# ningyu1991/InclusiveGAN

Hardware: AMD Instinct MI355X
Metric: training img/sec (whole node), CelebA 128x128 StyleGAN2+IMLE (higher is better)
Workload: dtype f32-equivalent (3x3 convs: 2-piece fp16 split, operands to <= 1 ulp of fp32, scales per pixel / per channel: no per-tensor window; fp32 sums)

## Files before the change

### include/igan_hip.h

```cpp
#ifndef IGAN_HIP_H
#define IGAN_HIP_H

#include <stddef.h>
#include <stdint.h>

#ifdef __cplusplus
extern "C" {
#endif

#define IGAN_ABI_VERSION 10

typedef void* igan_stream_t;

enum igan_status {
    IGAN_OK = 0,
    IGAN_ERR_INVALID_ARGUMENT = 1,
    IGAN_ERR_HIP = 2,
    IGAN_ERR_UNSUPPORTED = 3
};

int igan_abi_version(void);
size_t igan_struct_size(int which);
const char* igan_last_error(void);

// ... 89 lines not shown
    float* workspace;
    size_t workspace_floats;
    int N, H, W, Cin;
    int OH, OW, Cout;
    int KH, KW;
    int stride, up;
    int pad_y, pad_x;
    int splits;
    float alpha;
    const void* x_pieces;
    const void* dy_pieces;
    size_t x_pieces_bytes;
    size_t dy_pieces_bytes;
    const float* x_colmax;
    const float* dy_colmax;
} igan_conv2d_wgrad_params;

int igan_conv2d_wgrad_plan(const igan_conv2d_wgrad_params* p, int* splits, size_t* workspace_floats);
int igan_conv2d_wgrad(igan_stream_t stream, const igan_conv2d_wgrad_params* p);
int igan_conv2d_wgrad_kernel_name(const igan_conv2d_wgrad_params* p, char* buf, int buflen);

int igan_conv_pieces_wanted(int KH, int KW, int Cin, int Cout);
int igan_pieces_image_ok(int N, int HW, int C);
int igan_conv_piece_form(void);
size_t igan_filter_image_bytes(int KH, int KW, int Cin, int Cout);
int igan_filter_image(igan_stream_t stream, const float* w, void* out, int KH, int KW, int Cin, int Cout, int w_transposed);
#define IGAN_FILTER_MAX_GROUPS 48
typedef struct igan_filter_image_desc { const float* w; void* out; int KH, KW, Cin, Cout, w_transposed; } igan_filter_image_desc;
int igan_filter_images_grouped(igan_stream_t stream, const igan_filter_image_desc* groups, int count);
int igan_debug_filter_image_launches(unsigned long long* out, int reset);
size_t igan_colmax_floats(int N, int HW, int C);
int igan_debug_f16_window(unsigned long long* below, unsigned long long* imaged, int reset);
int igan_debug_f16_window_by_kind(unsigned long long* out4, int reset);

int igan_to_pieces(igan_stream_t stream, const float* x, const float* scale, void* out, int N, int HW, int C);

enum { IGAN_DENSE_PRO_NONE = 0, IGAN_DENSE_PRO_SQUARE = 1, IGAN_DENSE_PRO_DEMOD_GRAD = 2 };
enum { IGAN_DENSE_EPI_SCALE = 0, IGAN_DENSE_EPI_BIAS = 1, IGAN_DENSE_EPI_RSQRT = 2, IGAN_DENSE_EPI_STYLE_GRAD = 3 };
typedef struct igan_dense_params {
    const float* x;
    const float* x2;
    const float* w;
    float* y;
    const float* bias;
    const float* e1;
    const float* e2;
    float* colsum;
    int ldx, ldy;
    int M, K, N;
    int w_transposed;
    int prologue, epilogue;
    float alpha, pro_scale, bias_scale, add_const, eps;
} igan_dense_params;
int igan_dense_small(igan_stream_t stream, const igan_dense_params* p);

typedef struct igan_dense_wgrad_params {
    const float* a;
    const float* b;
    const float* b2;
    float* dw;
    int lda;
    int M, K, N;
    int pro_a, pro_b;
    float alpha, pro_scale;
} igan_dense_wgrad_params;
int igan_dense_small_wgrad(igan_stream_t stream, const igan_dense_wgrad_params* p);
// ... 192 lines not shown
```

### inclusivegan_amd/_abi.py

```python
import ctypes
import os
import threading

_HERE = os.path.dirname(os.path.abspath(__file__))
LIB_PATH = os.environ.get('IGAN_LIB') or os.path.join(_HERE, 'csrc', 'libigan_hip.so')

IGAN_OK = 0
IGAN_ERR_INVALID_ARGUMENT = 1
IGAN_ERR_HIP = 2
IGAN_ERR_UNSUPPORTED = 3

c_float_p = ctypes.POINTER(ctypes.c_float)


class UpFirDn2DParams(ctypes.Structure):
    _fields_ = [
        ('x', ctypes.c_void_p), ('k', ctypes.c_void_p), ('y', ctypes.c_void_p),
        ('upx', ctypes.c_int), ('upy', ctypes.c_int), ('downx', ctypes.c_int), ('downy', ctypes.c_int),
        ('padx0', ctypes.c_int), ('padx1', ctypes.c_int), ('pady0', ctypes.c_int), ('pady1', ctypes.c_int),
        ('majorDim', ctypes.c_int), ('inH', ctypes.c_int), ('inW', ctypes.c_int), ('minorDim', ctypes.c_int),
        ('kernelH', ctypes.c_int), ('kernelW', ctypes.c_int),
        ('outH', ctypes.c_int), ('outW', ctypes.c_int),
    ]

# ... 104 lines not shown

DENSE_MAX_GROUPS = 24
FILTER_MAX_GROUPS = 48
DENSE_PRO_NONE, DENSE_PRO_SQUARE, DENSE_PRO_DEMOD_GRAD = 0, 1, 2
DENSE_EPI_SCALE, DENSE_EPI_BIAS, DENSE_EPI_RSQRT, DENSE_EPI_STYLE_GRAD = 0, 1, 2, 3
DENSE_PRO_MUL = 3
DENSE_EPI_DEMOD_GRAD2, DENSE_EPI_STYLE_GRAD2 = 4, 5

_I, _F, _P, _SZ, _LL = ctypes.c_int, ctypes.c_float, ctypes.c_void_p, ctypes.c_size_t, ctypes.c_longlong

SIGNATURES = {
    'igan_abi_version': (_I, []),
    'igan_struct_size': (_SZ, [_I]),
    'igan_last_error': (ctypes.c_char_p, []),
    'igan_upfirdn2d': (_I, [_P, ctypes.POINTER(UpFirDn2DParams)]),
    'igan_upfirdn2d_f16': (_I, [_P, ctypes.POINTER(UpFirDn2DParams)]),
    'igan_upfirdn2d_ban': (_I, [_P, _P, _P, _P, _I, _P, _I, _F, _F]),
    'igan_fused_bias_act': (_I, [_P, ctypes.POINTER(FusedBiasActParams)]),
    'igan_fused_bias_act_f16': (_I, [_P, ctypes.POINTER(FusedBiasActParams)]),
    'igan_bias_grad_workspace_floats': (_SZ, [_I, _I, _I]),
    'igan_bias_grad': (_I, [_P, _P, _P, _P, _I, _I, _I]),
    'igan_bias_act_noise_workspace_floats': (_SZ, [_I, _I]),
    'igan_bias_act_noise_fwd': (_I, [_P, _P, _P, _P, _P, _P, _I, _I, _I, _F, _F]),
    'igan_bias_act_noise_dd_workspace_floats': (ctypes.c_size_t, [_I, _I, _I]),
    'igan_bias_act_noise_bwd_dd': (_I, [_P, _P, _P, _P, _P, _P, _P, _P, _P, _P, _P, _P, _I, _I, _I, _I, _I, _F, _F]),
    'igan_bias_act_noise_bwd': (_I, [_P, _P, _P, _P, _P, _P, _P, _P, _I, _I, _I, _F, _F]),
    'igan_conv2d_plan': (_I, [ctypes.POINTER(Conv2DParams), ctypes.POINTER(_I), ctypes.POINTER(_I), ctypes.POINTER(_SZ)]),
    'igan_conv2d': (_I, [_P, ctypes.POINTER(Conv2DParams)]),
    'igan_conv2d_kernel_name': (_I, [ctypes.POINTER(Conv2DParams), ctypes.c_char_p, _I]),
    'igan_conv2d_wgrad_kernel_name': (_I, [ctypes.POINTER(Conv2DWgradParams), ctypes.c_char_p, _I]),
    'igan_conv2d_wgrad_plan': (_I, [ctypes.POINTER(Conv2DWgradParams), ctypes.POINTER(_I), ctypes.POINTER(_SZ)]),
    'igan_conv2d_wgrad': (_I, [_P, ctypes.POINTER(Conv2DWgradParams)]),
    'igan_debug_f16_window_by_kind': (_I, [_P, _I]),
    'igan_colmax_floats': (ctypes.c_size_t, [_I, _I, _I]),
    'igan_filter_image_bytes': (ctypes.c_size_t, [_I, _I, _I, _I]),
    'igan_filter_image': (_I, [_P, _P, _P, _I, _I, _I, _I, _I]),
    'igan_filter_images_grouped': (_I, [_P, ctypes.POINTER(FilterImageDesc), _I]),
    'igan_debug_filter_image_launches': (_I, [_P, _I]),
    'igan_to_pieces': (_I, [_P, _P, _P, _P, _I, _I, _I]),
    'igan_conv_pieces_wanted': (_I, [_I, _I, _I, _I]),
    'igan_pieces_image_ok': (_I, [_I, _I, _I]),
    'igan_conv_piece_form': (_I, []),
    'igan_debug_f16_window': (_I, [_P, _P, _I]),
    'igan_dense_small': (_I, [_P, ctypes.POINTER(DenseParams)]),
    'igan_dense_small_wgrad': (_I, [_P, ctypes.POINTER(DenseWgradParams)]),
    'igan_dense_small_grouped': (_I, [_P, ctypes.POINTER(DenseParams), _I]),
    'igan_dense_small_wgrad_grouped': (_I, [_P, ctypes.POINTER(DenseWgradParams), _I]),
    'igan_dense_small2_grouped': (_I, [_P, ctypes.POINTER(Dense2Params), _I]),
    'igan_dense_small_wgrad2_grouped': (_I, [_P, ctypes.POINTER(DenseWgrad2Params), _I]),
    'igan_rows_group_sum': (_I, [_P, _P, ctypes.POINTER(ctypes.c_int), _I, _P, _I, _I, _I]),
    'igan_scale_add': (_I, [_P, _P, _P, _P, _P, _P, _I, _I, _I]),
    'igan_sumsq_taps_grouped': (_I, [_P, ctypes.POINTER(TapsParams), _I]),
    'igan_bcast_mul_taps_grouped': (_I, [_P, ctypes.POINTER(TapsParams), _I]),
    'igan_sumsq_taps': (_I, [_P, _P, _P, _I, _I]),
    'igan_bcast_mul_taps': (_I, [_P, _P, _P, _P, _I, _I, _F]),
    'igan_scale_dot_workspace_floats': (_SZ, [_I, _I, _I]),
    'igan_scale_dot': (_I, [_P, _P, _P, _P, _P, _P, _P, _I, _I, _I]),
    'igan_lpips_layer_blocks': (_I, [_I, _I]),
    'igan_lpips_layer_fwd': (_I, [_P, _P, _P, _P, _P, _I, _I, _I]),
    'igan_lpips_layer_bwd': (_I, [_P, _P, _P, _P, _P, _P, _I, _I, _I]),
    'igan_lpips_pairs_fwd': (_I, [_P, _P, _P, _P, _P, _P, _P, _I, _I, _I, _I, _I]),
    'igan_lpips_pairs_bwd': (_I, [_P, _P, _P, _P, _P, _P, _P, _P, _I, _I, _I, _I]),
    'igan_maxpool2x2_fwd': (_I, [_P, _P, _P, _I, _I, _I, _I]),
    'igan_maxpool2x2_bwd': (_I, [_P, _P, _P, _P, _P, _I, _I, _I, _I]),
    'igan_mbstd_workspace_floats': (_SZ, [_I, _I, _I, _I, _I]),
    'igan_mbstd_fwd': (_I, [_P, _P, _P, _P, _I, _I, _I, _I, _I]),
# ... 89 lines not shown
```

### inclusivegan_amd/csrc/conv2d_mfma.hip

```cpp
#include "igan_common.h"
#include <atomic>
#include <cmath>
#include <cstdlib>
#include <type_traits>

namespace {

typedef float f32x16 __attribute__((ext_vector_type(16)));

constexpr int BK = 32;
constexpr int LEAD_STEPS = 8;
constexpr int LDK = BK + 4;

struct ConvArgs {
    const float* x;
    const float* w;
    float* y;
    float* out;
    const float* in_scale;
    const float* out_scale;
    int N, H, W, Cin;
    int OH, OW, Cout;
    int KH, KW;
    int stride, up_shift;
    int pad_y, pad_x;
    int splits;
    int full_tiles;
    int nx, ny;
    int cpt;
    int Mtot;
    int vecA, vecB, vecS;
    int vecY;
    float alpha;
    int xcd_remap;
    int b_scale;
    int prio;
    int walk;
    int stagger;
    unsigned long long* diag;
    const float* bias;
    int act;
    float act_alpha, act_gain;
    const float* noise;
    const float* noise_strength;
    int noise_bcast;
    int diag_mode;
    const unsigned short* xp;
    const unsigned short* wp;
};

__device__ __forceinline__ float noise_term(const ConvArgs& a, int pix) {
    if (a.noise == nullptr || pix < 0) return 0.0f;
    return a.noise[a.noise_bcast ? pix % (a.OH * a.OW) : pix] * a.noise_strength[0];
}

__device__ __forceinline__ float epi_act(int act, float v, float alpha) {
    if (act == 2) return v > 0.f ? v : 0.f;
    if (act == 3) return v > 0.f ? v : v * alpha;
    return v;
}

__device__ __forceinline__ float4 f4zero() { return make_float4(0.f, 0.f, 0.f, 0.f); }
__device__ __forceinline__ float4 f4mul(float4 a, float4 b) { return make_float4(a.x * b.x, a.y * b.y, a.z * b.z, a.w * b.w); }
__device__ __forceinline__ float4 f4sel(bool has, float4 s) { return make_float4(has ? s.x : 1.f, has ? s.y : 1.f, has ? s.z : 1.f, has ? s.w : 1.f); }

typedef unsigned int u32x4 __attribute__((ext_vector_type(4)));
constexpr unsigned OOB = 0x7FFFFFF0u;

__device__ __forceinline__ __amdgpu_buffer_rsrc_t make_rsrc(const float* p, unsigned bytes) {
    return __builtin_amdgcn_make_buffer_rsrc(const_cast<float*>(p), 0, (int)bytes, 0x00020000);
}

struct LoadAddr {
    unsigned off;
    int left;
};
template <bool VEC>
__device__ __forceinline__ LoadAddr make_addr(int off, int left) {
    LoadAddr a;
    if constexpr (VEC) { a.off = (left > 0) ? (unsigned)off * 4u : OOB; a.left = 0; }
    else { a.off = (unsigned)off * 4u; a.left = left; }
// ... 890 lines not shown
    o[1] = __builtin_bit_cast(unsigned short, p1);
}

__device__ __forceinline__ void load_unit16(const float* __restrict__ x, const float* __restrict__ scale, int p, int c, int C, int HW, float (&v)[16]) {
    const float4* src = reinterpret_cast<const float4*>(x + (size_t)p * C + 16 * c);
#pragma unroll
    for (int i = 0; i < 4; i++) { const float4 f = src[i]; v[4 * i] = f.x; v[4 * i + 1] = f.y; v[4 * i + 2] = f.z; v[4 * i + 3] = f.w; }
    if (scale != nullptr) {
        const float4* sc = reinterpret_cast<const float4*>(scale + (size_t)(p / HW) * C + 16 * c);
#pragma unroll
        for (int i = 0; i < 4; i++) { const float4 f = sc[i]; v[4 * i] *= f.x; v[4 * i + 1] *= f.y; v[4 * i + 2] *= f.z; v[4 * i + 3] *= f.w; }
    }
}
__device__ __forceinline__ void store_units(const unsigned short (&pc)[2][16], uint4* stage, unsigned short* __restrict__ out, int total, int chunk) {
#pragma unroll
    for (int q = 0; q < 2; q++)
#pragma unroll
        for (int hh = 0; hh < 2; hh++) {
            uint4 u;
            u.x = pc[q][8 * hh + 0] | ((unsigned)pc[q][8 * hh + 1] << 16); u.y = pc[q][8 * hh + 2] | ((unsigned)pc[q][8 * hh + 3] << 16);
            u.z = pc[q][8 * hh + 4] | ((unsigned)pc[q][8 * hh + 5] << 16); u.w = pc[q][8 * hh + 6] | ((unsigned)pc[q][8 * hh + 7] << 16);
            stage[threadIdx.x * 4 + 2 * q + hh] = u;
        }
    __syncthreads();
    const int units = min(256, total - chunk * 256);
    uint4* dst = reinterpret_cast<uint4*>(out + (size_t)chunk * 256 * 32);
#pragma unroll
    for (int k = 0; k < 4; k++) {
        const int j = k * 256 + threadIdx.x;
        if (j < units * 4) dst[j] = stage[j];
    }
}

__global__ __launch_bounds__(256) void rows_f16_kernel(const float* __restrict__ x, const float* __restrict__ scale, unsigned short* __restrict__ out,
                                                        float* __restrict__ rowinv, float* __restrict__ colmax, int total, int cpp, int lcpp, int C, int HW) {
    __shared__ uint4 stage[256 * 4];
    const int c = threadIdx.x & (cpp - 1);
    float cm[16];
#pragma unroll
    for (int i = 0; i < 16; i++) cm[i] = 0.0f;
    int below = 0;
    const int nchunks = (total + 255) >> 8;
    for (int chunk = blockIdx.x; chunk < nchunks; chunk += gridDim.x) {
        const bool mine = chunk * 256 + (int)threadIdx.x < total;
        const int idx = min(chunk * 256 + (int)threadIdx.x, total - 1);
        const int p = idx >> lcpp;
        float v[16];
        load_unit16(x, scale, p, c, C, HW, v);
        float m = 0.0f;
#pragma unroll
        for (int i = 0; i < 16; i++) { const float av = fabsf(v[i]); m = fmaxf(m, av); if (mine) cm[i] = fmaxf(cm[i], av); }
        for (int o = 1; o < cpp; o <<= 1) m = fmaxf(m, __shfl_xor(m, o));
        const float S = scale_from_amax(m);
        if (mine && c == 0) rowinv[p] = inv_scale_from_amax(m);
        unsigned short pc[2][16];
#pragma unroll
        for (int i = 0; i < 16; i++) {
            unsigned short o[2];
            const float vs = v[i] * S;
            split2(vs, o);
            pc[0][i] = o[0]; pc[1][i] = o[1];
            below += (mine && vs != 0.0f && fabsf(vs) < 0x1p-12f) ? 1 : 0;
        }
        if (chunk != (int)blockIdx.x) __syncthreads();
        store_units(pc, stage, out, total, chunk);
    }
    count_window(below, &g_f16_below_window);
    if (blockIdx.x == 0 && threadIdx.x == 0) atomicAdd(&g_f16_imaged, (unsigned long long)total * 16ull);
    if (colmax != nullptr) {
        __syncthreads();
        float* sm = reinterpret_cast<float*>(stage);
#pragma unroll
        for (int i = 0; i < 16; i++) sm[threadIdx.x * 16 + i] = cm[i];
        __syncthreads();
        const int groups = 256 >> lcpp;
        for (int ch = threadIdx.x; ch < C; ch += 256) {
            const int cc = ch >> 4, i = ch & 15;
            float m = 0.0f;
            for (int j = 0; j < groups; j++) m = fmaxf(m, sm[(j * cpp + cc) * 16 + i]);
            colmax[4 + (size_t)blockIdx.x * C + ch] = m;
        }
        if (blockIdx.x == 0 && threadIdx.x == 0) colmax[0] = (float)gridDim.x;
    }
}

__global__ __launch_bounds__(256) void cols_amax_kernel(const float* __restrict__ x, const float* __restrict__ scale, float* __restrict__ partial,
                                                         int P_, int C4, int lC4, int HW, float* __restrict__ header) {
    if (header != nullptr && blockIdx.x == 0 && threadIdx.x == 0) header[0] = (float)gridDim.x;
    __shared__ float4 red[256];
    const int q = threadIdx.x & (C4 - 1), pl = threadIdx.x >> lC4, ppi = 256 >> lC4;
    const int step = gridDim.x * ppi;
    float4 m = make_float4(0.f, 0.f, 0.f, 0.f);
    auto take = [&](int p) {
        float4 v = reinterpret_cast<const float4*>(x)[(size_t)p * C4 + q];
        if (scale != nullptr) {
            const float4 f = reinterpret_cast<const float4*>(scale)[(size_t)(p / HW) * C4 + q];
            v.x *= f.x; v.y *= f.y; v.z *= f.z; v.w *= f.w;
        }
// ... 232 lines not shown
    const int py = cls >> a.up_shift, px = cls & (up - 1);
    const int QH = (a.OH - py + up - 1) >> a.up_shift;
    const int QW = (a.OW - px + up - 1) >> a.up_shift;
    const int Mcls = a.N * QH * QW;
    const int m0 = mt * BM;
    if (m0 >= Mcls) return;
    const int n0 = nt * BN;
    const int ky0 = (a.pad_y - py * a.stride) & (up - 1);
    const int kx0 = (a.pad_x - px * a.stride) & (up - 1);
    const int nky = (ky0 < a.KH) ? ((a.KH - ky0 + up - 1) >> a.up_shift) : 0;
    const int nkx = (kx0 < a.KW) ? ((a.KW - kx0 + up - 1) >> a.up_shift) : 0;
    const int chunks = nky * nkx * a.cpt;
    const int c_begin = sliced ? (int)(((long long)split * chunks) / nsplit) : 0;
    const int c_end = sliced ? (int)(((long long)(split + 1) * chunks) / nsplit) : chunks;

    const float inv_hw = 1.0f / (float)(QH * QW), inv_w = 1.0f / (float)QW;
    const int drow = 32 * (wave & 3) + (lane >> 1);
    const int dhalf = (lane & 1) ^ ((drow >> 3) & 1);
    const bool lowave = wave < 4;
    const int ntap = nky * nkx;
    int ld_cc, ld_t0;
    if constexpr (TAPO) {
        ld_t0 = (c_begin < c_end) ? c_begin / a.cpt : 0;
        ld_cc = (c_begin < c_end) ? c_begin - ld_t0 * a.cpt : 0;
    } else {
        ld_cc = (c_begin < c_end) ? c_begin / ntap : 0;
        ld_t0 = (c_begin < c_end) ? c_begin - ld_cc * ntap : 0;
    }
    int ld_ta = (c_begin < c_end) ? ld_t0 / nkx : 0;
    int ld_tb = (c_begin < c_end) ? ld_t0 - ld_ta * nkx : 0;
    const unsigned xbytes = (unsigned)a.N * a.H * a.W * a.Cin * (2u * NP), wbytes = (unsigned)a.KH * a.KW * a.Cin * a.Cout * (2u * NP);
    const __amdgpu_buffer_rsrc_t rx = __builtin_amdgcn_make_buffer_rsrc(const_cast<unsigned short*>(a.xp), 0, (int)xbytes, 0x00020000);
    const __amdgpu_buffer_rsrc_t rw = __builtin_amdgcn_make_buffer_rsrc(const_cast<unsigned short*>(a.wp), 0, (int)wbytes, 0x00020000);
    const unsigned pixA = (unsigned)a.Cin * (2u * NP);
    unsigned baseA, maskA = 0u, voffB;
    {
        const int m = m0 + drow;
        const bool rok = m < Mcls;
        const int mm = rok ? m : 0;
        const int nn = div_small(mm, QH * QW, inv_hw);
        const int r = mm - nn * (QH * QW);
        const int qy = div_small(r, QW, inv_w), qx = r - qy * QW;
        const int vy0 = (qy * up + py) * a.stride - a.pad_y + ky0, vx0 = (qx * up + px) * a.stride - a.pad_x + kx0;
        const int iy0 = vy0 >> a.up_shift, ix0 = vx0 >> a.up_shift;
        baseA = (unsigned)((nn * a.H + iy0) * a.W + ix0) * pixA + (unsigned)dhalf * 16u;
        for (int ta = 0; ta < nky; ta++)
            for (int tb = 0; tb < nkx; tb++) {
                const int iy = iy0 + ta, ix = ix0 + tb;
                const bool ok = rok & (iy >= 0) & (ix >= 0) & (iy < a.H) & (ix < a.W);
                maskA |= ok ? (1u << (ta * nkx + tb)) : 0u;
            }
        const int co = n0 + drow;
        voffB = (co < a.Cout) ? (unsigned)co * PB + (unsigned)dhalf * 16u : OOB;
    }
    unsigned offA = OOB, soffB = 0u;
    typedef __attribute__((address_space(3))) void lds_void;
    unsigned char* dA = nullptr;
    bool dma_fresh = true;
    const unsigned sliceB = (unsigned)(a.KH * a.KW * a.Cout) * PB;
    auto dma_prep = [&](int stage) {
        if (!TAPO || dma_fresh || ld_cc == 0) {
            const unsigned disp = (unsigned)(ld_ta * a.W + ld_tb) * pixA + (unsigned)ld_cc * PB;
            const unsigned bit = 1u << (ld_ta * nkx + ld_tb);
            offA = (maskA & bit) ? baseA + disp : OOB;
            const int ky = ky0 + (ld_ta << a.up_shift), kx = kx0 + (ld_tb << a.up_shift);
            soffB = __builtin_amdgcn_readfirstlane((unsigned)((ld_cc * (a.KH * a.KW) + ky * a.KW + kx) * a.Cout) * PB);
            dma_fresh = false;
        } else {
            offA += PB;
            soffB = __builtin_amdgcn_readfirstlane(soffB + sliceB);
        }
        dA = smem + stage * STAGE + (wave & 3) * 1024;
        if constexpr (TAPO) {
            ++ld_cc;
            const int w1 = (ld_cc == a.cpt) ? 1 : 0;
            ld_cc = w1 ? 0 : ld_cc;
            ld_tb += w1;
            const int w2 = (ld_tb == nkx) ? 1 : 0;
            ld_tb = w2 ? 0 : ld_tb;
            ld_ta += w2;
        } else {
            ++ld_tb;
            const int w1 = (ld_tb == nkx) ? 1 : 0;
            ld_tb = w1 ? 0 : ld_tb;
            ld_ta += w1;
            const int w2 = (ld_ta == nky) ? 1 : 0;
            ld_ta = w2 ? 0 : ld_ta;
            ld_cc += w2;
        }
    };
    auto dma_piece = [&](int j) {
        unsigned char* A = dA;
        unsigned char* B = dA + IMG;
        if constexpr (NP == 2) {
            const unsigned sB = __builtin_amdgcn_readfirstlane(soffB);
            if (lowave) {
                if (j == 0) __builtin_amdgcn_raw_ptr_buffer_load_lds(rx, (lds_void*)A, 16, offA, 0, 0, 0);
                if (j == 1) __builtin_amdgcn_raw_ptr_buffer_load_lds(rw, (lds_void*)(B + 4096), 16, voffB, sB + 32u, 0, 0);
            } else {
                if (j == 0) __builtin_amdgcn_raw_ptr_buffer_load_lds(rx, (lds_void*)(A + 4096), 16, offA, 32, 0, 0);
                if (j == 1) __builtin_amdgcn_raw_ptr_buffer_load_lds(rw, (lds_void*)B, 16, voffB, sB, 0, 0);
            }
        } else
        if (lowave) {
            if (j == 0) __builtin_amdgcn_raw_ptr_buffer_load_lds(rx, (lds_void*)A, 16, offA, 0, 0, 0);
            if (j == 1) __builtin_amdgcn_raw_ptr_buffer_load_lds(rx, (lds_void*)(A + 2 * 4096), 16, offA, 64, 0, 0);
            if (j == 2) __builtin_amdgcn_raw_ptr_buffer_load_lds(rw, (lds_void*)(B + 4096), 16, voffB, soffB + 32u, 0, 0);
        } else {
            if (j == 0) __builtin_amdgcn_raw_ptr_buffer_load_lds(rx, (lds_void*)(A + 4096), 16, offA, 32, 0, 0);
            if (j == 1) __builtin_amdgcn_raw_ptr_buffer_load_lds(rw, (lds_void*)B, 16, voffB, soffB, 0, 0);
            if (j == 2) __builtin_amdgcn_raw_ptr_buffer_load_lds(rw, (lds_void*)(B + 2 * 4096), 16, voffB, soffB + 64u, 0, 0);
        }
    };
    auto dma_chunk = [&](int stage) { dma_prep(stage); dma_piece(0); dma_piece(1); if constexpr (NP == 3) dma_piece(2); };

    f32x16 acc[TM];
#pragma unroll
    for (int tm = 0; tm < TM; tm++)
#pragma unroll
        for (int r = 0; r < 16; r++) acc[tm][r] = 0.0f;

    float tabv[3] = {0.0f, 0.0f, 0.0f};
    if constexpr (NP == 2) {
        const float* rowinv = reinterpret_cast<const float*>(reinterpret_cast<const unsigned char*>(a.xp) + (size_t)a.N * a.H * a.W * a.Cin * 4);
#pragma unroll
        for (int j = 0; j < 3; j++) {
            const int i = tid + 512 * j;
            const int t = i >> 7, r = i & 127;
            if (t < ntap) {
                const int ta = t / nkx, tb = t - ta * nkx;
                const int m = m0 + r;
                const bool rok = m < Mcls;
                const int mm = rok ? m : 0;
                const int nn = div_small(mm, QH * QW, inv_hw);
                const int rr = mm - nn * (QH * QW);
                const int qy = div_small(rr, QW, inv_w), qx = rr - qy * QW;
                const int iy = (((qy * up + py) * a.stride - a.pad_y + ky0) >> a.up_shift) + ta, ix = (((qx * up + px) * a.stride - a.pad_x + kx0) >> a.up_shift) + tb;
                if (rok & (iy >= 0) & (ix >= 0) & (iy < a.H) & (ix < a.W)) tabv[j] = rowinv[(nn * a.H + iy) * a.W + ix];
            }
        }
    }
    if (c_begin < c_end) { dma_chunk(0); dma_chunk(1); }
// ... 491 lines not shown
    const bool sliced = bid >= a.full_tiles;
    const int tail = bid - a.full_tiles;
    const int tile = sliced ? a.full_tiles + tail / a.splits : bid;
    const int split = sliced ? tail % a.splits : 0;
    const int nsplit = sliced ? a.splits : 1;
    const int mt = tile % a.nx, nt = (tile / a.nx) % a.ny, cls = tile / (a.nx * a.ny);
    const int py = cls >> a.up_shift, px = cls & (up - 1);
    const int QH = (a.OH - py + up - 1) >> a.up_shift;
    const int QW = (a.OW - px + up - 1) >> a.up_shift;
    const int Mcls = a.N * QH * QW;
    const int m0 = mt * BM;
    if (m0 >= Mcls) return;
    const int n0 = nt * BN;
    const int ky0 = (a.pad_y - py * a.stride) & (up - 1);
    const int kx0 = (a.pad_x - px * a.stride) & (up - 1);
    const int nky = (ky0 < a.KH) ? ((a.KH - ky0 + up - 1) >> a.up_shift) : 0;
    const int nkx = (kx0 < a.KW) ? ((a.KW - kx0 + up - 1) >> a.up_shift) : 0;
    const int chunks = nky * nkx * a.cpt;
    const int c_begin = sliced ? (int)(((long long)split * chunks) / nsplit) : 0;
    const int c_end = sliced ? (int)(((long long)(split + 1) * chunks) / nsplit) : chunks;
    const bool any = c_begin < c_end;

    const float inv_hw = 1.0f / (float)(QH * QW), inv_w = 1.0f / (float)QW;
    const int drow = 32 * wave + (lane >> 1);
    const int dhalf = (lane & 1) ^ ((drow >> 3) & 1);
    const int ntap = nky * nkx;
    int ld_t0 = any ? c_begin / a.cpt : 0;
    int ld_cc = any ? c_begin - ld_t0 * a.cpt : 0;
    int ld_ta = any ? ld_t0 / nkx : 0;
    int ld_tb = any ? ld_t0 - ld_ta * nkx : 0;
    const unsigned xbytes = (unsigned)a.N * a.H * a.W * a.Cin * 4u, wbytes = (unsigned)a.KH * a.KW * a.Cin * a.Cout * 4u;
    const __amdgpu_buffer_rsrc_t rx = __builtin_amdgcn_make_buffer_rsrc(const_cast<unsigned short*>(a.xp), 0, (int)xbytes, 0x00020000);
    const __amdgpu_buffer_rsrc_t rw = __builtin_amdgcn_make_buffer_rsrc(const_cast<unsigned short*>(a.wp), 0, (int)wbytes, 0x00020000);
    const unsigned pixA = (unsigned)a.Cin * 4u;
    unsigned baseA, maskA = 0u, voffB;
    {
        const int m = m0 + drow;
        const bool rok = m < Mcls;
        const int mm = rok ? m : 0;
        const int nn = div_small(mm, QH * QW, inv_hw);
        const int r = mm - nn * (QH * QW);
        const int qy = div_small(r, QW, inv_w), qx = r - qy * QW;
        const int vy0 = (qy * up + py) * a.stride - a.pad_y + ky0, vx0 = (qx * up + px) * a.stride - a.pad_x + kx0;
        const int iy0 = vy0 >> a.up_shift, ix0 = vx0 >> a.up_shift;
        baseA = (unsigned)((nn * a.H + iy0) * a.W + ix0) * pixA + (unsigned)dhalf * 16u;
        for (int ta = 0; ta < nky; ta++)
            for (int tb = 0; tb < nkx; tb++) {
                const int iy = iy0 + ta, ix = ix0 + tb;
                const bool ok = rok & (iy >= 0) & (ix >= 0) & (iy < a.H) & (ix < a.W);
                maskA |= ok ? (1u << (ta * nkx + tb)) : 0u;
            }
        const int co = n0 + drow;
        voffB = (co < a.Cout) ? (unsigned)co * PB + (unsigned)dhalf * 16u : OOB;
    }
    unsigned offA = OOB, soffB = 0u;
    typedef __attribute__((address_space(3))) void lds_void;
    bool dma_fresh = true;
    const unsigned sliceB = (unsigned)(a.KH * a.KW * a.Cout) * PB;
    auto dma_prep = [&]() {
        if (dma_fresh || ld_cc == 0) {
            const unsigned disp = (unsigned)(ld_ta * a.W + ld_tb) * pixA + (unsigned)ld_cc * PB;
            const unsigned bit = 1u << (ld_ta * nkx + ld_tb);
            offA = (maskA & bit) ? baseA + disp : OOB;
            const int ky = ky0 + (ld_ta << a.up_shift), kx = kx0 + (ld_tb << a.up_shift);
            soffB = __builtin_amdgcn_readfirstlane((unsigned)((ld_cc * (a.KH * a.KW) + ky * a.KW + kx) * a.Cout) * PB);
            dma_fresh = false;
        } else {
            offA += PB;
            soffB = __builtin_amdgcn_readfirstlane(soffB + sliceB);
        }
        ++ld_cc;
        const int w1 = (ld_cc == a.cpt) ? 1 : 0;
        ld_cc = w1 ? 0 : ld_cc;
        ld_tb += w1;
        const int w2 = (ld_tb == nkx) ? 1 : 0;
        ld_tb = w2 ? 0 : ld_tb;
        ld_ta += w2;
    };
    auto dma_pair = [&](int stage, int which) {
        unsigned char* D = smem + stage * STAGE + wave * 1024;
        if (which == 0) {
            __builtin_amdgcn_raw_ptr_buffer_load_lds(rx, (lds_void*)D, 16, offA, 0, 0, 0);
            __builtin_amdgcn_raw_ptr_buffer_load_lds(rx, (lds_void*)(D + 4096), 16, offA, 32, 0, 0);
        } else {
            const unsigned sB = __builtin_amdgcn_readfirstlane(soffB);
            __builtin_amdgcn_raw_ptr_buffer_load_lds(rw, (lds_void*)(D + IMG), 16, voffB, sB, 0, 0);
            __builtin_amdgcn_raw_ptr_buffer_load_lds(rw, (lds_void*)(D + IMG + 4096), 16, voffB, sB + 32u, 0, 0);
        }
    };

    f32x16 acc[2][2];
#pragma unroll
    for (int i = 0; i < 2; i++)
#pragma unroll
        for (int j = 0; j < 2; j++)
#pragma unroll
            for (int r = 0; r < 16; r++) acc[i][j][r] = 0.0f;

    float tabv[5] = {0.0f, 0.0f, 0.0f, 0.0f, 0.0f};
    {
        const float* rowinv = reinterpret_cast<const float*>(reinterpret_cast<const unsigned char*>(a.xp) + (size_t)a.N * a.H * a.W * a.Cin * 4);
#pragma unroll
        for (int j = 0; j < 5; j++) {
            const int i = tid + 256 * j;
            const int t = i >> 7, r = i & 127;
            if (t < ntap) {
                const int ta = t / nkx, tb = t - ta * nkx;
                const int m = m0 + r;
                const bool rok = m < Mcls;
                const int mm = rok ? m : 0;
                const int nn = div_small(mm, QH * QW, inv_hw);
                const int rr = mm - nn * (QH * QW);
                const int qy = div_small(rr, QW, inv_w), qx = rr - qy * QW;
                const int iy = (((qy * up + py) * a.stride - a.pad_y + ky0) >> a.up_shift) + ta, ix = (((qx * up + px) * a.stride - a.pad_x + kx0) >> a.up_shift) + tb;
                if (rok & (iy >= 0) & (ix >= 0) & (iy < a.H) & (ix < a.W)) tabv[j] = rowinv[(nn * a.H + iy) * a.W + ix];
            }
// ... 550 lines not shown
    static const bool dma = !(getenv("IGAN_CONV_DMA") && atoi(getenv("IGAN_CONV_DMA")) == 0);
    if (!dma || t.BM != 128 || t.BN != 128 || !walk) return false;
    if ((long long)p->N * p->OH * p->OW >= (1LL << 24)) return false;
    if (p->in_scale) {
        const int up = p->up;
        for (int c = 0; c < up * up; c++) {
            const int qh = (p->OH - c / up + up - 1) / up, qw = (p->OW - c % up + up - 1) / up;
            if (qh <= 0 || qw <= 0) continue;
            const int samples = 127 / (qh * qw) + 2;
            if ((long long)std::min(samples, p->N) * p->Cin > 2048) return false;
        }
    }
    return true;
}

bool xcd_remap_on() {
    static const bool remap = !(getenv("IGAN_XCD_REMAP") && atoi(getenv("IGAN_XCD_REMAP")) == 0);
    return remap;
}

int planes_mode() {
    static const int mode = [] { const char* v = getenv("IGAN_CONV_PLANES"); const int m = v ? atoi(v) : 2; return m == 0 ? 0 : (m == 1 ? 1 : 2); }();
    return mode;
}
bool planes_enabled() { return planes_mode() != 0; }

int ilog2(int v) { int l = 0; while ((1 << l) < v) ++l; return l; }
bool pow2(int v) { return v > 0 && (v & (v - 1)) == 0; }

void launch_piece_image(hipStream_t stream, const float* x, const float* scale, unsigned short* out, int P_, int HW, int C) {
    const int cpp = C / PK, total = P_ * cpp;
    hipLaunchKernelGGL(to_planes_kernel, dim3(igan::ceil_div(total, 256)), dim3(256), 0, stream, x, scale, out, total, cpp, C, HW);
}
void launch_row_image(hipStream_t stream, const float* x, const float* scale, unsigned short* out, int P_, int HW, int C, float* colmax) {
    const int cpp = C / PK, total = P_ * cpp;
    float* rowinv = reinterpret_cast<float*>(reinterpret_cast<unsigned char*>(out) + (size_t)P_ * C * 4);
    const int nchunks = igan::ceil_div(total, 256);
    const int grid = colmax ? std::min(nchunks, H_COLBLOCKS) : nchunks;
    hipLaunchKernelGGL(rows_f16_kernel, dim3(grid), dim3(256), 0, stream, x, scale, out, rowinv, colmax, total, cpp, ilog2(cpp), C, HW);
}
void launch_colmax_only(hipStream_t stream, const float* x, const float* scale, float* colmax, int P_, int HW, int C) {
    const int C4 = C / 4, ppi = 256 / C4;
    const int blocks = std::min(H_COLBLOCKS, igan::ceil_div(P_, ppi));
    hipLaunchKernelGGL(cols_amax_kernel, dim3(blocks), dim3(256), 0, stream, x, scale, colmax + 4, P_, C4, ilog2(C4), HW, colmax);
}
void launch_col_image(hipStream_t stream, const float* x, const float* scale, unsigned short* out, int P_, int HW, int C, const float* colmax) {
    const int cpp = C / PK, total = P_ * cpp, C4 = C / 4;
    float* inv = reinterpret_cast<float*>(reinterpret_cast<unsigned char*>(out) + (size_t)P_ * C * 4);
    float* sc = inv + C;
    float* partial = sc + C;
    const int ppi = 256 / C4;
    const int blocks = std::min(H_COLBLOCKS, igan::ceil_div(P_, ppi));
    if (colmax == nullptr) {
        hipLaunchKernelGGL(cols_amax_kernel, dim3(blocks), dim3(256), 0, stream, x, scale, partial, P_, C4, ilog2(C4), HW, (float*)nullptr);
        hipLaunchKernelGGL(cols_finalize_kernel, dim3(igan::ceil_div(C, 8)), dim3(256), 0, stream, (const float*)partial, inv, sc, blocks, C, (const float*)nullptr);
    } else
        hipLaunchKernelGGL(cols_finalize_kernel, dim3(igan::ceil_div(C, 8)), dim3(256), 0, stream, colmax + 4, inv, sc, 0, C, colmax);
    hipLaunchKernelGGL(cols_f16_kernel, dim3(igan::ceil_div(total, 256)), dim3(256), 0, stream, x, scale, out, (const float*)sc, total, cpp, C, HW);
}
bool f16_w4() { static const int v = getenv("IGAN_F16_W4") ? atoi(getenv("IGAN_F16_W4")) : 1; return v != 0; }
std::atomic<unsigned long long> g_filter_image_launches{0ull};
void launch_filter_image(hipStream_t stream, const float* w, unsigned short* wp, bool wt, int taps, int KW_, int Nn, int K) {
    const int wtotal = taps * Nn * (K / PK);
    g_filter_image_launches += planes_mode() == 2 ? 2ull : 1ull;
    if (planes_mode() == 2) {
        float* inv = reinterpret_cast<float*>(reinterpret_cast<unsigned char*>(wp) + (size_t)taps * Nn * K * 4);
        float* partial = inv + Nn;
        if (wt) {
            hipLaunchKernelGGL((filter_amax_kernel<true>), dim3(igan::ceil_div(taps * Nn, 4)), dim3(256), 0, stream, w, partial, taps, Nn, K);
            hipLaunchKernelGGL((filter_planes_f16_kernel<true>), dim3(igan::ceil_div(wtotal, 256)), dim3(256), 0, stream, w, wp, inv, (const float*)partial, taps, taps, KW_, Nn, K);
        } else {
            hipLaunchKernelGGL((filter_amax_kernel<false>), dim3(taps * H_KSK, igan::ceil_div(Nn, 64)), dim3(256), 0, stream, w, partial, taps, Nn, K);
// ... 51 lines not shown
    bool piece_room;
};
bool is_piece_family(FwdFamily f) { return f == FWD_PIECES_W4 || f == FWD_PIECES_W8 || f == FWD_PIECES_BF16; }

FwdChoice choose_fwd(const igan_conv2d_params* p) {
    FwdChoice c = {};
    if (is_small_dense(p)) { c.family = c.fp32_family = FWD_DENSE_SMALL; return c; }
    if (const int kind = igan::thin_conv_kind(p)) { c.family = c.fp32_family = FWD_THIN; c.thin_kind = kind; return c; }
    fwd_counts(p, c.Mmax, c.chunks_max, c.nclass);
    c.t = pick_fwd_tile(c.Mmax, p->Cout);
    c.wt = p->w_transposed != 0;
    c.sc = p->in_scale != nullptr;
    c.vecA = (p->Cin % 4 == 0) && (((uintptr_t)p->x & 15) == 0);
    c.vecS = (p->Cin % 4 == 0) && (((uintptr_t)p->in_scale & 15) == 0);
    c.vecB = ((c.wt ? p->Cin : p->Cout) % 4 == 0) && (((uintptr_t)p->w & 15) == 0);
    c.vec = c.vecA && c.vecB && (!c.sc || c.vecS);
    c.walk = c.vec && (p->Cin % BK == 0);
    c.wm = 2; c.wn = 4;
    if (c.t.BM == 128 && c.t.BN == 64) { c.wm = 4; c.wn = 2; }
    if (c.t.BM == 128 && c.t.BN == 32) { c.wm = 4; c.wn = 1; }
    if (c.t.BM == 32) { c.wm = 1; c.wn = 4; }
    c.fp32_family = use_dma_kernel(p, c.t, c.walk) ? FWD_DMA : FWD_TILE;
    c.piece_room = planes_shape_ok(p, c.t, c.Mmax);
    if (c.piece_room && planes_operands_aligned(p)) c.family = (planes_mode() != 2) ? FWD_PIECES_BF16 : (f16_w4() ? FWD_PIECES_W4 : FWD_PIECES_W8);
    else c.family = c.fp32_family;
    return c;
}


}

static unsigned long long* g_conv_diag = nullptr;
extern "C" void igan_debug_set_conv_diag(unsigned long long* p) { g_conv_diag = p; }

static int conv2d_plan_tiles(const igan_conv2d_params* p, const FwdChoice& c, int* splits, int* sliced_tiles, size_t* workspace_floats);

extern "C" int igan_conv2d_plan(const igan_conv2d_params* p, int* splits, int* sliced_tiles, size_t* workspace_floats) {
    IGAN_REQUIRE(p && splits && sliced_tiles && workspace_floats, "conv2d_plan: null argument");
    if (int rc = fwd_geometry_check(p)) return rc;
    *splits = 1;
    *sliced_tiles = 0;
    *workspace_floats = 0;
    const FwdChoice c = choose_fwd(p);
    if (c.family == FWD_DENSE_SMALL || c.family == FWD_THIN) return IGAN_OK;
    if (int rc = conv2d_plan_tiles(p, c, splits, sliced_tiles, workspace_floats)) return rc;
    if (c.piece_room)
        *workspace_floats += planes_x_floats(p) + planes_w_floats(p);
    return IGAN_OK;
}

static int conv2d_plan_tiles(const igan_conv2d_params* p, const FwdChoice& c, int* splits, int* sliced_tiles, size_t* workspace_floats) {
    const int chunks_max = c.chunks_max;
    const FwdTile t = c.t;
    const TileList l = tile_list(p, t, c.Mmax, c.nclass);
    if (l.rem == 0) return IGAN_OK;
    const int cus = device_cus();
    const double shape = (t.BM == 128 ? 1.0 : 0.4) * (t.BN / 128.0 > 0.5 ? 1.0 : 0.5);
    const double t2 = chunks_max * 4.4e-6 * shape, t1 = chunks_max * 3.3e-6 * shape;
    auto pairs = [&](int n) { return (n / 2) * t2 + (n % 2) * t1; };
    const double bw = 4.0e12;
    const int cand[] = {2, 3, 4, 5, 6, 7, 8, 10, 12, 14, 16, 20, 24, 32, 48, 64};
    int best_s = 1, best_sl = 0;
    double best = pairs(igan::ceil_div(l.T, cus));
    for (int k = 0; k <= std::min(l.T / cus, 3); k++) {
        const int sl = l.rem + k * cus;
        if (sl == 0) continue;
// ... 70 lines not shown
        IGAN_REQUIRE(p->workspace != nullptr, "conv2d: splits > 1 needs a workspace");
        IGAN_REQUIRE(p->workspace_floats >= partial_floats, "conv2d: workspace too small");
    }
    if (splits > 1 || planes) IGAN_REQUIRE((((uintptr_t)p->workspace) & 15) == 0, "conv2d: workspace must be 16-byte aligned");

    ConvArgs a;
    a.x = p->x; a.w = p->w;
    a.y = (splits > 1) ? p->workspace : nullptr;
    a.out = p->y;
    a.in_scale = p->in_scale; a.out_scale = p->out_scale;
    a.N = p->N; a.H = p->H; a.W = p->W; a.Cin = p->Cin;
    a.OH = p->OH; a.OW = p->OW; a.Cout = p->Cout;
    a.KH = p->KH; a.KW = p->KW;
    a.stride = p->stride; a.up_shift = (p->up == 2) ? 1 : 0;
    a.pad_y = p->pad_y; a.pad_x = p->pad_x;
    a.splits = splits;
    a.nx = l.nx; a.ny = l.ny;
    a.full_tiles = (splits > 1) ? l.T - sliced : l.T;
    a.cpt = ceil_div(p->Cin, BK);
    a.Mtot = p->N * p->OH * p->OW;
    a.vecA = c.vecA; a.vecB = c.vecB; a.vecS = c.vecS;
    a.vecY = (p->Cout % 2 == 0) && ((((uintptr_t)p->y | (uintptr_t)p->out_scale) & 7) == 0);
    a.alpha = p->alpha;
    a.xcd_remap = xcd_remap_on() ? 1 : 0;
    a.walk = c.walk ? 1 : 0;
    a.diag = g_conv_diag;
    a.stagger = 0;
    a.b_scale = 1;
    a.prio = 1;
    a.diag_mode = 0;
    a.bias = p->bias; a.act = p->act; a.act_alpha = p->act_alpha; a.act_gain = p->act_gain;
    a.noise = p->act ? p->noise : nullptr; a.noise_strength = p->noise_strength; a.noise_bcast = p->noise_bcast;
    a.xp = nullptr; a.wp = nullptr;

    dim3 grid(a.full_tiles + (l.T - a.full_tiles) * splits);
    if (!planes) colmax_own_pass();
    if (planes) {
        IGAN_REQUIRE(p->x_pieces == nullptr || planes_mode() == 1, "conv2d: the two-piece fp16 form writes its own images (one scale per pixel here, per channel in the weight gradient): x_pieces must be NULL");
        IGAN_REQUIRE(p->x_pieces == nullptr || p->x_pieces_bytes == planes_x_floats(p) * 4, "conv2d: x_pieces is not the image of this x (x_pieces_bytes != N*H*W*Cin*6)");
        const unsigned short* xp = reinterpret_cast<const unsigned short*>(p->x_pieces);
        unsigned short* wp = reinterpret_cast<unsigned short*>(p->workspace + partial_floats + planes_x_floats(p));
        if (xp == nullptr) {
            unsigned short* own = reinterpret_cast<unsigned short*>(p->workspace + partial_floats);
            if (planes_mode() == 2) launch_row_image(stream, p->x, p->in_scale, own, p->N * p->H * p->W, p->H * p->W, p->Cin, p->x_colmax);
            else launch_piece_image(stream, p->x, p->in_scale, own, p->N * p->H * p->W, p->H * p->W, p->Cin);
            xp = own;
        }
        if (p->w_pieces != nullptr) {
            IGAN_REQUIRE(p->w_pieces_bytes == igan_filter_image_bytes(p->KH, p->KW, p->Cin, p->Cout) && (((uintptr_t)p->w_pieces) & 15) == 0,
                         "conv2d: w_pieces is not an image igan_filter_image() wrote for this filter (size / alignment)");
            wp = reinterpret_cast<unsigned short*>(const_cast<void*>(p->w_pieces));
        } else launch_filter_image(stream, p->w, wp, c.wt, p->KH * p->KW, p->KW, p->Cout, p->Cin);
        a.xp = xp; a.wp = wp;
        a.cpt = p->Cin / PK;
    }
    switch (family) {
    case FWD_PIECES_W4:
        hipLaunchKernelGGL(conv_fwd_planes_w4_kernel, grid, dim3(256), 0, stream, a);
        IGAN_LAUNCH_CHECK("conv2d (piece form) launch");
        break;
    case FWD_PIECES_W8:
        hipLaunchKernelGGL((conv_fwd_planes_kernel<2, true>), grid, dim3(512), 0, stream, a);
        IGAN_LAUNCH_CHECK("conv2d (piece form) launch");
        break;
    case FWD_PIECES_BF16:
        hipLaunchKernelGGL((conv_fwd_planes_kernel<3>), grid, dim3(512), 0, stream, a);
        IGAN_LAUNCH_CHECK("conv2d (piece form) launch");
        break;
    case FWD_DMA:
        if (c.wt) {
            if (c.sc) hipLaunchKernelGGL((conv_fwd_dma_kernel<true, true>), grid, dim3(512), 0, stream, a);
            else hipLaunchKernelGGL((conv_fwd_dma_kernel<true, false>), grid, dim3(512), 0, stream, a);
        } else {
            if (c.sc) hipLaunchKernelGGL((conv_fwd_dma_kernel<false, true>), grid, dim3(512), 0, stream, a);
            else hipLaunchKernelGGL((conv_fwd_dma_kernel<false, false>), grid, dim3(512), 0, stream, a);
        }
        IGAN_LAUNCH_CHECK("conv2d (LDS-DMA) launch");
// ... 380 lines not shown
```

Before: 359.5.

## Add slice-major layout for two-piece fp16 row image in stride-1 convs

Adds a planar (slice-major) layout for the per-pixel two-piece fp16 activation image: 32-byte channel slices of all pixels are stored contiguously per slice and per piece instead of interleaved per pixel. The row-image kernel gains a planar store path through a padded LDS stage, and the forward conv kernels now take pixel, slice and piece strides from the args rather than hardcoded offsets. By default it is enabled for stride-1 convs and can be changed with an environment variable or a debug setter. The aim is more contiguous, better-coalesced buffer-to-LDS loads of A tiles. The cost is a different write pattern and extra LDS padding in the image kernel, and any other consumer of x_pieces must agree on the layout.

```diff
diff --git a/include/igan_hip.h b/include/igan_hip.h
--- a/include/igan_hip.h
+++ b/include/igan_hip.h
@@ -145,6 +145,8 @@
 size_t igan_colmax_floats(int N, int HW, int C);
 int igan_debug_f16_window(unsigned long long* below, unsigned long long* imaged, int reset);
 int igan_debug_f16_window_by_kind(unsigned long long* out4, int reset);
+int igan_debug_set_row_image_layout(int layout);
+int igan_debug_row_image_strides(long long P, int C, int layout, unsigned* out3);
 
 int igan_to_pieces(igan_stream_t stream, const float* x, const float* scale, void* out, int N, int HW, int C);
 
diff --git a/inclusivegan_amd/_abi.py b/inclusivegan_amd/_abi.py
--- a/inclusivegan_amd/_abi.py
+++ b/inclusivegan_amd/_abi.py
@@ -160,6 +160,8 @@
     'igan_conv2d_wgrad_plan': (_I, [ctypes.POINTER(Conv2DWgradParams), ctypes.POINTER(_I), ctypes.POINTER(_SZ)]),
     'igan_conv2d_wgrad': (_I, [_P, ctypes.POINTER(Conv2DWgradParams)]),
     'igan_debug_f16_window_by_kind': (_I, [_P, _I]),
+    'igan_debug_set_row_image_layout': (_I, [_I]),
+    'igan_debug_row_image_strides': (_I, [_LL, _I, _I, _P]),
     'igan_colmax_floats': (ctypes.c_size_t, [_I, _I, _I]),
     'igan_filter_image_bytes': (ctypes.c_size_t, [_I, _I, _I, _I]),
     'igan_filter_image': (_I, [_P, _P, _P, _I, _I, _I, _I, _I]),
diff --git a/inclusivegan_amd/csrc/conv2d_mfma.hip b/inclusivegan_amd/csrc/conv2d_mfma.hip
--- a/inclusivegan_amd/csrc/conv2d_mfma.hip
+++ b/inclusivegan_amd/csrc/conv2d_mfma.hip
@@ -47,6 +47,7 @@
     int diag_mode;
     const unsigned short* xp;
     const unsigned short* wp;
+    unsigned a_pix, a_slice, a_piece;
 };
 
 __device__ __forceinline__ float noise_term(const ConvArgs& a, int pix) {
@@ -1003,9 +1004,35 @@
     }
 }
 
+constexpr int STAGE_PLANAR = 256 * 4 + 64;
+__device__ __forceinline__ void store_units_planar(const unsigned short (&pc)[2][16], uint4* stage, unsigned short* __restrict__ out, int total, int chunk, int cpp, int lcpp) {
+    const int lppc = 8 - lcpp;
+    const int c = threadIdx.x & (cpp - 1), pl = threadIdx.x >> lcpp;
+#pragma unroll
+    for (int q = 0; q < 2; q++)
+#pragma unroll
+        for (int hh = 0; hh < 2; hh++) {
+            uint4 u;
+            u.x = pc[q][8 * hh + 0] | ((unsigned)pc[q][8 * hh + 1] << 16); u.y = pc[q][8 * hh + 2] | ((unsigned)pc[q][8 * hh + 3] << 16);
+            u.z = pc[q][8 * hh + 4] | ((unsigned)pc[q][8 * hh + 5] << 16); u.w = pc[q][8 * hh + 6] | ((unsigned)pc[q][8 * hh + 7] << 16);
+            stage[((((2 * c + q) << lppc) + pl) << 1) + hh + c] = u;
+        }
+    __syncthreads();
+    const int P_ = total >> lcpp, p0 = chunk << lppc;
+    const int lrun = lppc + 1;
+    uint4* dst = reinterpret_cast<uint4*>(out);
+#pragma unroll
+    for (int k = 0; k < 4; k++) {
+        const int j = k * 256 + threadIdx.x;
+        const int r = j >> lrun, within = j & ((1 << lrun) - 1);
+        if (p0 + (within >> 1) < P_) dst[(((size_t)r * P_ + p0) << 1) + within] = stage[j + (r >> 1)];
+    }
+}
+
+template <bool PLANAR>
 __global__ __launch_bounds__(256) void rows_f16_kernel(const float* __restrict__ x, const float* __restrict__ scale, unsigned short* __restrict__ out,
                                                         float* __restrict__ rowinv, float* __restrict__ colmax, int total, int cpp, int lcpp, int C, int HW) {
-    __shared__ uint4 stage[256 * 4];
+    __shared__ uint4 stage[PLANAR ? STAGE_PLANAR : 256 * 4];
     const int c = threadIdx.x & (cpp - 1);
     float cm[16];
 #pragma unroll
@@ -1034,7 +1061,8 @@
             below += (mine && vs != 0.0f && fabsf(vs) < 0x1p-12f) ? 1 : 0;
         }
         if (chunk != (int)blockIdx.x) __syncthreads();
-        store_units(pc, stage, out, total, chunk);
+        if constexpr (PLANAR) store_units_planar(pc, stage, out, total, chunk, cpp, lcpp);
+        else store_units(pc, stage, out, total, chunk);
     }
     count_window(below, &g_f16_below_window);
     if (blockIdx.x == 0 && threadIdx.x == 0) atomicAdd(&g_f16_imaged, (unsigned long long)total * 16ull);
@@ -1333,7 +1361,7 @@
     const unsigned xbytes = (unsigned)a.N * a.H * a.W * a.Cin * (2u * NP), wbytes = (unsigned)a.KH * a.KW * a.Cin * a.Cout * (2u * NP);
     const __amdgpu_buffer_rsrc_t rx = __builtin_amdgcn_make_buffer_rsrc(const_cast<unsigned short*>(a.xp), 0, (int)xbytes, 0x00020000);
     const __amdgpu_buffer_rsrc_t rw = __builtin_amdgcn_make_buffer_rsrc(const_cast<unsigned short*>(a.wp), 0, (int)wbytes, 0x00020000);
-    const unsigned pixA = (unsigned)a.Cin * (2u * NP);
+    const unsigned pixA = a.a_pix, sliceA = a.a_slice, pieceA = __builtin_amdgcn_readfirstlane(a.a_piece);
     unsigned baseA, maskA = 0u, voffB;
     {
         const int m = m0 + drow;
@@ -1361,14 +1389,14 @@
     const unsigned sliceB = (unsigned)(a.KH * a.KW * a.Cout) * PB;
     auto dma_prep = [&](int stage) {
         if (!TAPO || dma_fresh || ld_cc == 0) {
-            const unsigned disp = (unsigned)(ld_ta * a.W + ld_tb) * pixA + (unsigned)ld_cc * PB;
+            const unsigned disp = (unsigned)(ld_ta * a.W + ld_tb) * pixA + (unsigned)ld_cc * sliceA;
             const unsigned bit = 1u << (ld_ta * nkx + ld_tb);
             offA = (maskA & bit) ? baseA + disp : OOB;
             const int ky = ky0 + (ld_ta << a.up_shift), kx = kx0 + (ld_tb << a.up_shift);
             soffB = __builtin_amdgcn_readfirstlane((unsigned)((ld_cc * (a.KH * a.KW) + ky * a.KW + kx) * a.Cout) * PB);
             dma_fresh = false;
         } else {
-            offA += PB;
+            offA += sliceA;
             soffB = __builtin_amdgcn_readfirstlane(soffB + sliceB);
         }
         dA = smem + stage * STAGE + (wave & 3) * 1024;
@@ -1399,16 +1427,16 @@
                 if (j == 0) __builtin_amdgcn_raw_ptr_buffer_load_lds(rx, (lds_void*)A, 16, offA, 0, 0, 0);
                 if (j == 1) __builtin_amdgcn_raw_ptr_buffer_load_lds(rw, (lds_void*)(B + 4096), 16, voffB, sB + 32u, 0, 0);
             } else {
-                if (j == 0) __builtin_amdgcn_raw_ptr_buffer_load_lds(rx, (lds_void*)(A + 4096), 16, offA, 32, 0, 0);
+                if (j == 0) __builtin_amdgcn_raw_ptr_buffer_load_lds(rx, (lds_void*)(A + 4096), 16, offA, pieceA, 0, 0);
                 if (j == 1) __builtin_amdgcn_raw_ptr_buffer_load_lds(rw, (lds_void*)B, 16, voffB, sB, 0, 0);
             }
         } else
         if (lowave) {
             if (j == 0) __builtin_amdgcn_raw_ptr_buffer_load_lds(rx, (lds_void*)A, 16, offA, 0, 0, 0);
-            if (j == 1) __builtin_amdgcn_raw_ptr_buffer_load_lds(rx, (lds_void*)(A + 2 * 4096), 16, offA, 64, 0, 0);
+            if (j == 1) __builtin_amdgcn_raw_ptr_buffer_load_lds(rx, (lds_void*)(A + 2 * 4096), 16, offA, 2u * pieceA, 0, 0);
             if (j == 2) __builtin_amdgcn_raw_ptr_buffer_load_lds(rw, (lds_void*)(B + 4096), 16, voffB, soffB + 32u, 0, 0);
         } else {
-            if (j == 0) __builtin_amdgcn_raw_ptr_buffer_load_lds(rx, (lds_void*)(A + 4096), 16, offA, 32, 0, 0);
+            if (j == 0) __builtin_amdgcn_raw_ptr_buffer_load_lds(rx, (lds_void*)(A + 4096), 16, offA, pieceA, 0, 0);
             if (j == 1) __builtin_amdgcn_raw_ptr_buffer_load_lds(rw, (lds_void*)B, 16, voffB, soffB, 0, 0);
             if (j == 2) __builtin_amdgcn_raw_ptr_buffer_load_lds(rw, (lds_void*)(B + 2 * 4096), 16, voffB, soffB + 64u, 0, 0);
         }
@@ -1966,7 +1994,7 @@
     const unsigned xbytes = (unsigned)a.N * a.H * a.W * a.Cin * 4u, wbytes = (unsigned)a.KH * a.KW * a.Cin * a.Cout * 4u;
     const __amdgpu_buffer_rsrc_t rx = __builtin_amdgcn_make_buffer_rsrc(const_cast<unsigned short*>(a.xp), 0, (int)xbytes, 0x00020000);
     const __amdgpu_buffer_rsrc_t rw = __builtin_amdgcn_make_buffer_rsrc(const_cast<unsigned short*>(a.wp), 0, (int)wbytes, 0x00020000);
-    const unsigned pixA = (unsigned)a.Cin * 4u;
+    const unsigned pixA = a.a_pix, sliceA = a.a_slice, pieceA = a.a_piece;
     unsigned baseA, maskA = 0u, voffB;
     {
         const int m = m0 + drow;
@@ -1993,14 +2021,14 @@
     const unsigned sliceB = (unsigned)(a.KH * a.KW * a.Cout) * PB;
     auto dma_prep = [&]() {
         if (dma_fresh || ld_cc == 0) {
-            const unsigned disp = (unsigned)(ld_ta * a.W + ld_tb) * pixA + (unsigned)ld_cc * PB;
+            const unsigned disp = (unsigned)(ld_ta * a.W + ld_tb) * pixA + (unsigned)ld_cc * sliceA;
             const unsigned bit = 1u << (ld_ta * nkx + ld_tb);
             offA = (maskA & bit) ? baseA + disp : OOB;
             const int ky = ky0 + (ld_ta << a.up_shift), kx = kx0 + (ld_tb << a.up_shift);
             soffB = __builtin_amdgcn_readfirstlane((unsigned)((ld_cc * (a.KH * a.KW) + ky * a.KW + kx) * a.Cout) * PB);
             dma_fresh = false;
         } else {
-            offA += PB;
+            offA += sliceA;
             soffB = __builtin_amdgcn_readfirstlane(soffB + sliceB);
         }
         ++ld_cc;
@@ -2015,7 +2043,7 @@
         unsigned char* D = smem + stage * STAGE + wave * 1024;
         if (which == 0) {
             __builtin_amdgcn_raw_ptr_buffer_load_lds(rx, (lds_void*)D, 16, offA, 0, 0, 0);
-            __builtin_amdgcn_raw_ptr_buffer_load_lds(rx, (lds_void*)(D + 4096), 16, offA, 32, 0, 0);
+            __builtin_amdgcn_raw_ptr_buffer_load_lds(rx, (lds_void*)(D + 4096), 16, offA, __builtin_amdgcn_readfirstlane(pieceA), 0, 0);
         } else {
             const unsigned sB = __builtin_amdgcn_readfirstlane(soffB);
             __builtin_amdgcn_raw_ptr_buffer_load_lds(rw, (lds_void*)(D + IMG), 16, voffB, sB, 0, 0);
@@ -2632,12 +2660,27 @@
     const int cpp = C / PK, total = P_ * cpp;
     hipLaunchKernelGGL(to_planes_kernel, dim3(igan::ceil_div(total, 256)), dim3(256), 0, stream, x, scale, out, total, cpp, C, HW);
 }
-void launch_row_image(hipStream_t stream, const float* x, const float* scale, unsigned short* out, int P_, int HW, int C, float* colmax) {
+void launch_row_image(hipStream_t stream, const float* x, const float* scale, unsigned short* out, int P_, int HW, int C, float* colmax, int layout) {
     const int cpp = C / PK, total = P_ * cpp;
     float* rowinv = reinterpret_cast<float*>(reinterpret_cast<unsigned char*>(out) + (size_t)P_ * C * 4);
     const int nchunks = igan::ceil_div(total, 256);
     const int grid = colmax ? std::min(nchunks, H_COLBLOCKS) : nchunks;
-    hipLaunchKernelGGL(rows_f16_kernel, dim3(grid), dim3(256), 0, stream, x, scale, out, rowinv, colmax, total, cpp, ilog2(cpp), C, HW);
+    if (layout == 1) hipLaunchKernelGGL(rows_f16_kernel<true>, dim3(grid), dim3(256), 0, stream, x, scale, out, rowinv, colmax, total, cpp, ilog2(cpp), C, HW);
+    else hipLaunchKernelGGL(rows_f16_kernel<false>, dim3(grid), dim3(256), 0, stream, x, scale, out, rowinv, colmax, total, cpp, ilog2(cpp), C, HW);
+}
+std::atomic<int> g_row_image_layout{-1};
+int row_image_layout(const igan_conv2d_params* p) {
+    int v = g_row_image_layout.load(std::memory_order_relaxed);
+    if (v < 0) {
+        const char* e = getenv("IGAN_ROW_IMAGE");
+        v = e ? (atoi(e) == 0 ? 0 : 1) : 2;
+        g_row_image_layout.store(v, std::memory_order_relaxed);
+    }
+    return v == 2 ? (p->stride == 1 ? 1 : 0) : v;
+}
+void row_image_strides(size_t P_, int C, int pieces, int layout, unsigned (&s)[3]) {
+    if (layout == 1) { s[0] = 32u; s[1] = (unsigned)(P_ * 32u * pieces); s[2] = (unsigned)(P_ * 32u); }
+    else { s[0] = (unsigned)C * 2u * pieces; s[1] = 32u * pieces; s[2] = 32u; }
 }
 void launch_colmax_only(hipStream_t stream, const float* x, const float* scale, float* colmax, int P_, int HW, int C) {
     const int C4 = C / 4, ppi = 256 / C4;
@@ -2755,6 +2798,22 @@
 
 static unsigned long long* g_conv_diag = nullptr;
 extern "C" void igan_debug_set_conv_diag(unsigned long long* p) { g_conv_diag = p; }
+
+extern "C" int igan_debug_set_row_image_layout(int layout) {
+    IGAN_REQUIRE(layout == 0 || layout == 1, "debug_set_row_image_layout: layout must be 0 (pixel-major) or 1 (slice-major)");
+    g_row_image_layout.store(layout, std::memory_order_relaxed);
+    return IGAN_OK;
+}
+extern "C" int igan_debug_row_image_strides(long long P, int C, int layout, unsigned* out3) {
+    IGAN_REQUIRE(out3 != nullptr, "debug_row_image_strides: null argument");
+    IGAN_REQUIRE(layout == 0 || layout == 1, "debug_row_image_strides: layout must be 0 (pixel-major) or 1 (slice-major)");
+    IGAN_REQUIRE(P >= 1 && C >= 16 && C % 16 == 0, "debug_row_image_strides: P >= 1 pixels of a positive multiple of 16 channels");
+    IGAN_REQUIRE(P * C * 6 < 0x7FFFFF00LL, "debug_row_image_strides: image too large (planes_shape_ok: 32-bit offsets)");
+    unsigned s[3];
+    row_image_strides((size_t)P, C, 2, layout, s);
+    out3[0] = s[0]; out3[1] = s[1]; out3[2] = s[2];
+    return IGAN_OK;
+}
 
 static int conv2d_plan_tiles(const igan_conv2d_params* p, const FwdChoice& c, int* splits, int* sliced_tiles, size_t* workspace_floats);
 
@@ -2891,6 +2950,7 @@
     a.bias = p->bias; a.act = p->act; a.act_alpha = p->act_alpha; a.act_gain = p->act_gain;
     a.noise = p->act ? p->noise : nullptr; a.noise_strength = p->noise_strength; a.noise_bcast = p->noise_bcast;
     a.xp = nullptr; a.wp = nullptr;
+    a.a_pix = a.a_slice = a.a_piece = 0u;
 
     dim3 grid(a.full_tiles + (l.T - a.full_tiles) * splits);
     if (!planes) colmax_own_pass();
@@ -2899,9 +2959,13 @@
         IGAN_REQUIRE(p->x_pieces == nullptr || p->x_pieces_bytes == planes_x_floats(p) * 4, "conv2d: x_pieces is not the image of this x (x_pieces_bytes != N*H*W*Cin*6)");
         const unsigned short* xp = reinterpret_cast<const unsigned short*>(p->x_pieces);
         unsigned short* wp = reinterpret_cast<unsigned short*>(p->workspace + partial_floats + planes_x_floats(p));
+        const int layout = (planes_mode() == 2) ? row_image_layout(p) : 0;
+        unsigned steps[3];
+        row_image_strides((size_t)p->N * p->H * p->W, p->Cin, planes_mode() == 2 ? 2 : 3, layout, steps);
+        a.a_pix = steps[0]; a.a_slice = steps[1]; a.a_piece = steps[2];
         if (xp == nullptr) {
             unsigned short* own = reinterpret_cast<unsigned short*>(p->workspace + partial_floats);
-            if (planes_mode() == 2) launch_row_image(stream, p->x, p->in_scale, own, p->N * p->H * p->W, p->H * p->W, p->Cin, p->x_colmax);
+            if (planes_mode() == 2) launch_row_image(stream, p->x, p->in_scale, own, p->N * p->H * p->W, p->H * p->W, p->Cin, p->x_colmax, layout);
             else launch_piece_image(stream, p->x, p->in_scale, own, p->N * p->H * p->W, p->H * p->W, p->Cin);
             xp = own;
         }
```

After: 361.7 (median of 6 runs). Within noise of the previous version (+0.6%).
